# PRBonn/lidar_transfer

Hardware: AMD Instinct MI355X
Metric: Mrays/sec, one new ~1M-triangle mesh per scan -> 64x2048 range/label image (higher is better)
Workload: dtype f32; 1 GPU; C2: 64x2048 rays vs 999788-triangle synthetic scene (fov 3.0/-25.0); 1 step = 64 scans, each a new mesh; 48 scenes cycled; parallelism=scan-parallel x1, scans_in_flight=24, scans_per_call=8

## Files before the change

### lidar_transfer_amd/csrc/lt_api.hip

```cpp
#include "lt_internal.h"
#include <cpuid.h>
#include <stdarg.h>
#include <stdlib.h>
#include <string.h>

static thread_local char g_err[512] = "";

void lt_set_error(const char* fmt, ...) {
  va_list ap;
  va_start(ap, fmt);
  vsnprintf(g_err, sizeof(g_err), fmt, ap);
  va_end(ap);
}

int lt_cu_count(int device) {
  static int cache[64];
  const int slot = (device >= 0 && device < 64) ? device : 0;
  int v = __atomic_load_n(&cache[slot], __ATOMIC_RELAXED);
  if (v > 0) return v;
  hipDeviceProp_t prop;
  v = (hipGetDeviceProperties(&prop, device) == hipSuccess && prop.multiProcessorCount > 0) ? prop.multiProcessorCount : 256;
  __atomic_store_n(&cache[slot], v, __ATOMIC_RELAXED);
  return v;
}
// ... 77 lines not shown
  if (!out) {
    lt_set_error("lt_scene_create: NULL out pointer");
    return LT_ERR_INVALID_ARG;
  }
  *out = nullptr;
  if (device < 0) LT_HIP(hipGetDevice(&device));
  LT_HIP(hipSetDevice(device));
  lt_scene* s = (lt_scene*)calloc(1, sizeof(lt_scene));
  if (!s) {
    lt_set_error("lt_scene_create: out of host memory");
    return LT_ERR_NO_MEMORY;
  }
  s->device = device;
  int rc = dev_alloc(&s->partial, 6 * LT_BOUNDS_BLOCKS);
  if (rc == LT_OK) rc = dev_alloc(&s->params, 8);
  if (rc == LT_OK) rc = dev_alloc(&s->flags, 4);
  if (rc == LT_OK) rc = dev_alloc(&s->counters, 8 + 4 * LT_DBG_WAVES);
  if (rc == LT_OK && hipMemset(s->flags, 0, 4 * sizeof(unsigned)) != hipSuccess) rc = LT_ERR_HIP;
  for (int k = 0; rc == LT_OK && k < 10; ++k) {
    if (hipEventCreate(&s->ev[k]) != hipSuccess) {
      lt_set_error("hipEventCreate failed");
      rc = LT_ERR_HIP;
    } else {
      s->have_events = k + 1;
    }
  }
  if (rc != LT_OK) {
    lt_scene_destroy(s);
    return rc;
  }
  *out = s;
  return LT_OK;
}

extern "C" int lt_scene_destroy(lt_scene* s) {
  if (!s) return LT_OK;
  (void)hipSetDevice(s->device);
  (void)hipDeviceSynchronize();
  ws_free(s);
  if (s->owned_mesh) (void)hipFree(s->owned_mesh);
  if (s->partial) (void)hipFree(s->partial);
  if (s->params) (void)hipFree(s->params);
  if (s->flags) (void)hipFree(s->flags);
  if (s->counters) (void)hipFree(s->counters);
  if (s->overflow) (void)hipFree(s->overflow);
  if (s->tail_stack) (void)hipFree(s->tail_stack);
  if (s->tail_meta) (void)hipFree(s->tail_meta);
  if (s->tail_queue) (void)hipFree(s->tail_queue);
  if (s->tail_count) (void)hipFree(s->tail_count);
  if (s->sc_cell) (void)hipFree(s->sc_cell);
  if (s->sc_large) (void)hipFree(s->sc_large);
  if (s->sc_slices) (void)hipFree(s->sc_slices);
  if (s->sc_large_count) (void)hipFree(s->sc_large_count);
  for (int k = 0; k < s->have_events; ++k) (void)hipEventDestroy(s->ev[k]);
  free(s);
  return LT_OK;
}

int lt_check_mesh_args(const char* who, const void* verts, const void* faces, const void* colors,
                           const void* rem, int n_verts, int n_faces) {
  if (n_verts < 0 || n_faces < 0 || (n_faces > 0 && (!verts || !faces || !colors || !rem))) {
    lt_set_error("%s: invalid mesh (n_verts=%d n_faces=%d, NULL array?)", who, n_verts, n_faces);
    return LT_ERR_INVALID_ARG;
  }
  if (n_faces >= LT_MAX_FACES) {
    lt_set_error("%s: %d faces exceed LT_MAX_FACES", who, n_faces);
    return LT_ERR_TOO_LARGE;
  }
  return LT_OK;
}

extern "C" int lt_scene_set_mesh_dev(lt_scene* s, const float* verts, const int* faces, const int* colors,
                                     const float* rem, int n_verts, int n_faces) {
  if (!s) {
    lt_set_error("lt_scene_set_mesh_dev: NULL scene");
    return LT_ERR_INVALID_ARG;
  }
  LT_CHECK(lt_check_mesh_args("lt_scene_set_mesh_dev", verts, faces, colors, rem, n_verts, n_faces));
  s->verts = verts; s->faces = faces; s->colors = colors; s->rem = rem;
  s->n_verts = n_verts; s->n_faces = n_faces;
  s->built = 0;
  return LT_OK;
}

static size_t align256(size_t x) { return (x + 255) & ~(size_t)255; }

extern "C" int lt_scene_set_mesh_host(lt_scene* s, const float* verts, const int* faces, const int* colors,
                                      const float* rem, int n_verts, int n_faces, void* stream_) {
  if (!s) {
    lt_set_error("lt_scene_set_mesh_host: NULL scene");
    return LT_ERR_INVALID_ARG;
  }
  LT_CHECK(lt_check_mesh_args("lt_scene_set_mesh_host", verts, faces, colors, rem, n_verts, n_faces));
  hipStream_t stream = (hipStream_t)stream_;
  LT_HIP(hipSetDevice(s->device));
  const size_t bv = align256((size_t)n_verts * 12), bf = align256((size_t)n_faces * 12), bc = bv,
               br = align256((size_t)n_verts * 4);
  const size_t total = bv + bf + bc + br + 256;
  if (total > s->owned_mesh_bytes) {
    if (s->owned_mesh) {
      LT_HIP(hipDeviceSynchronize());
      (void)hipFree(s->owned_mesh);
      s->owned_mesh = nullptr;
      s->owned_mesh_bytes = 0;
    }
    LT_HIP(hipMalloc(&s->owned_mesh, total + total / 4));
// ... 156 lines not shown
```

### lidar_transfer_amd/csrc/lt_internal.h

```cpp
#pragma once
#include <hip/hip_runtime.h>
#include <stdint.h>
#include <stdio.h>
#include "lidarhip.h"

void lt_set_error(const char* fmt, ...);
int lt_cu_count(int device);

#define LT_HIP(call)                                                                          \
  do {                                                                                        \
    hipError_t e__ = (call);                                                                  \
    if (e__ != hipSuccess) {                                                                  \
      lt_set_error("%s failed: %s (%s:%d)", #call, hipGetErrorString(e__), __FILE__, __LINE__); \
      return e__ == hipErrorOutOfMemory ? LT_ERR_NO_MEMORY : LT_ERR_HIP;                      \
    }                                                                                         \
  } while (0)

#define LT_CHECK(expr)              \
  do {                              \
    int rc__ = (expr);              \
    if (rc__ != LT_OK) return rc__; \
  } while (0)

#define LT_FOR_MODEL(rows, sector, az, LAUNCH)                           \
// ... 7 lines not shown
                double fov_down_deg, int H, const double* sec, const double* az, int n_az, double* tab);
bool sector_ok(const char* who, double yaw_center, double span);
bool beam_azimuth_ok(const char* who, const double* az, int n);


#define LT_LEAF_MAX 4
#ifndef LT_SORT_TILE
#define LT_SORT_TILE 4096
#endif
#define LT_SORT_THREADS 256
#define LT_SEG_SUB 512
#define LT_STACK_LDS 32
#define LT_STACK_MAX 64
#define LT_STACK4_LDS 40
#define LT_STACK4_MAX 104
#define LT_TAIL_SAVE (LT_STACK4_MAX + 1)
#define LT_TAIL_STACK 512
#define LT_TAIL_DFS 256
#define LT_TRACE4_STEP_CAP 40

struct lt_scene {
  int device;
  const float* verts;
  const int* faces;
  const int* colors;
  const float* rem;
  int n_verts, n_faces;
  void* owned_mesh;
  size_t owned_mesh_bytes;
  int cap_faces;
  int np;
  uint32_t* keys[2];
  uint32_t* vals[2];
  uint32_t* hist;
  float4* tris;
  float4* seg;
  float4* nodes;
  float4* nodes4;
  float* partial;
  float* params;
  unsigned* flags;
  unsigned long long* counters;
  int* overflow;
  int cap_rays;
  int* tail_stack;
  float4* tail_meta;
  int* tail_queue;
  int* tail_count;
  int tail_parity;
  unsigned long long* sc_cell;
  int* sc_large;
  int2* sc_slices;
  int* sc_large_count;
  int sc_cap_cells, sc_cap_queue;
  int built;
  int sorted_buf;
  hipStream_t last_stream;
  hipEvent_t probe[2];
  hipEvent_t ev[10];
  int have_events;
  lt_stats stats;
};

struct lt_tsdf {
  int device;
  int dim[3];
  float origin[3];
  float voxel_size, trunc_margin;
  double voxel_size_d;
  double fov_up_deg, fov_down_deg;
  double bnds_given[6];
  size_t n;
  float *tsdf, *weight, *color, *rem;
  unsigned* col_epoch;
  unsigned* col_zw;
  unsigned epoch;
  int all_dirty;
  unsigned long long* bits;
  int* colinfo;
  float* colmax;
  int cap_w;
  int walk_w;
  float2* dct;
  size_t cap_dct;
  int n_obs;
  int wd_w;
  int wd_rho_bits, wd_n_quirk;
  float wd_qscale;
  int* wd_px;
  int* wd_start;
  int2* wd_ent;
  unsigned* wd_key;
  unsigned* wd_qcols;
  float4* rowtab;
  int rowtab_h;
  int rowtab_for_h;
  unsigned* zw_snap;
  unsigned* chunk_epoch;
  float4* obs4;
  size_t cap_obs4;
};

#define LT_BOUNDS_BLOCKS 256
#define LT_DBG_WAVES 16384
#define LT_FLAG_BAD_INDEX 1u
#define LT_FLAG_HIER_OVERFLOW 2u
#define LT_TRACE_DEBUG_STEPS 0x4000u
// ... 37 lines not shown
```

### lidar_transfer_amd/csrc/lt_scatter.hip

```cpp
#include "lt_internal.h"
#include <math.h>
#include <type_traits>
#include <stdlib.h>
#include <string.h>
#include "lt_normalize.h"

#define LT_PI_F 3.14159265358979f
#define LT_BIN_SLACK 4e-3f
#define LT_EMPTY_KEY 0xFFFFFFFFFFFFFFFFull

struct rs_params {
  int nb_az, nb_el;
  float az_scale;
  float az_off;
  float el_lo, el_scale;
  float dev_az, dev_el;
  float dev_fit[2];
  float el_c0, el_c1, az_c0, az_c1;
};

__device__ __forceinline__ float rs_az_off(float phi0, float az_scale) {
  if (!(phi0 == phi0)) return 0.f;
  const float x0 = (phi0 + LT_PI_F) * az_scale;
  return x0 - floorf(x0 + 0.5f);
}

__global__ __launch_bounds__(256) void k_rs_dirs(const float* __restrict__ rays, int n, unsigned flags,
                                                 float4* __restrict__ dirs, float2* __restrict__ ang,
                                                 float* __restrict__ partial) {
  __shared__ float red[4][2];
  float lo = INFINITY, hi = -INFINITY;
  for (int i = blockIdx.x * 256 + threadIdx.x; i < n; i += gridDim.x * 256) {
    const float rx = rays[3 * (size_t)i], ry = rays[3 * (size_t)i + 1], rz = rays[3 * (size_t)i + 2];
    const float D = (rx * rx + ry * ry) + rz * rz;
    const float r0 = lt_rsqrt_seed(D, flags);
    const float r = (1.5f * r0) + (((D * -0.5f) * r0) * (r0 * r0));
    const float dx = rx * r, dy = ry * r, dz = rz * r;
    dirs[i] = make_float4(dx, dy, dz, 0.f);
    const float phi = atan2f(dy, dx), th = atan2f(dz, sqrtf(dx * dx + dy * dy));
    ang[i] = make_float2(phi, th);
    if (th == th) { lo = fminf(lo, th); hi = fmaxf(hi, th); }
  }
#pragma unroll
  for (int o = 32; o > 0; o >>= 1) {
    lo = fminf(lo, __shfl_xor(lo, o, 64));
    hi = fmaxf(hi, __shfl_xor(hi, o, 64));
  }
  if ((threadIdx.x & 63) == 0) { red[threadIdx.x >> 6][0] = lo; red[threadIdx.x >> 6][1] = hi; }
  __syncthreads();
  if (threadIdx.x == 0) {
    partial[2 * blockIdx.x] = fminf(fminf(red[0][0], red[1][0]), fminf(red[2][0], red[3][0]));
    partial[2 * blockIdx.x + 1] = fmaxf(fmaxf(red[0][1], red[1][1]), fmaxf(red[2][1], red[3][1]));
  }
}
// ... 273 lines not shown
    n_tests += w >= 0 ? 1u : 0u;
    sc_hit<WIDE>(sc_mt(T, ox, oy, oz, g.x, g.y, g.z), w, face, cell);
  } else {
    for (int k = __float_as_int(g.x), e = __float_as_int(g.y); k < e; ++k) {
      const float4 d = *at<WIDE>(sdirs, (unsigned)k);
      ++n_tests;
      sc_hit<WIDE>(sc_mt(T, ox, oy, oz, d.x, d.y, d.z), __float_as_int(d.w), face, cell);
    }
  }
}

__global__ __launch_bounds__(256) void k_rs_sortdirs(const float4* __restrict__ dirs,
                                                     const uint32_t* __restrict__ bin_rays, int n,
                                                     float4* __restrict__ sdirs) {
  const int k = blockIdx.x * 256 + threadIdx.x;
  if (k >= n) return;
  const int ray = (int)bin_rays[k];
  float4 d = dirs[ray];
  d.w = __int_as_float(ray);
  sdirs[k] = d;
}

__global__ __launch_bounds__(256) void k_rs_grid(const int* __restrict__ bin_start,
                                                 const float4* __restrict__ sdirs, int nbins,
                                                 float4* __restrict__ grid) {
  const int b = blockIdx.x * 256 + threadIdx.x;
  if (b >= nbins) return;
  const int s = bin_start[b], e = bin_start[b + 1];
  float4 g = make_float4(0.f, 0.f, 0.f, __int_as_float(LT_GRID_EMPTY));
  if (e - s == 1) g = sdirs[s];
  else if (e - s > 1) g = make_float4(__int_as_float(s), __int_as_float(e), 0.f, __int_as_float(LT_GRID_MULTI));
  grid[b] = g;
}

#define LT_SC_BIG 512
#define LT_SC_CAP_SINGLE 1536
#define LT_SC_CAP_BATCH 8192
#ifndef LT_SC_SLICE
#define LT_SC_SLICE 512
#endif

#ifndef LT_SC_T
#define LT_SC_T 448
#endif
#define LT_SC_T2 (LT_SC_T - 256)
static_assert(LT_SC_T >= 256 && LT_SC_T <= 512 && LT_SC_T2 % 64 == 0, "LT_SC_T: 256, 320, 384, 448 or 512");

struct sc_shared {
  float4 q0[LT_SC_T], q1[LT_SC_T];
  float2 q2[LT_SC_T];
  unsigned pre[513];
  unsigned wsum[4];
  int kept;
};

struct sc_one { int cnt; unsigned a0; };

template <bool PUSH>
__device__ __forceinline__ sc_one sc_record_into(float4* s_q0, float4* s_q1, float2* s_q2, int slot, int f, const f3 A,
                                                 const f3 Bv, const f3 C, float ox, float oy, float oz, const rs_params& P,
                                                 int* __restrict__ large, int* __restrict__ large_count) {
  sc_one r;
  r.cnt = 0; r.a0 = 0;
  const float v0x = A.x, v0y = A.y, v0z = A.z, v1x = Bv.x, v1y = Bv.y, v1z = Bv.z;
  const float v2x = C.x, v2y = C.y, v2z = C.z;
  const float e1x = v1x - v0x, e1y = v1y - v0y, e2x = v2x - v0x, e2y = v2y - v0y;
  const bin_rect R = tri_bins(P, v0x - ox, v0y - oy, v0z - oz, v1x - ox, v1y - oy, v1z - oz, v2x - ox, v2y - oy,
                              v2z - oz, e1x, e1y, e2x, e2y);
  if (R.na > 0) {
    const int c32 = R.na * (R.e1 - R.e0 + 1);
    if (c32 > LT_SC_BIG) {
      if (PUSH) large[atomicAdd(large_count, 1)] = f;
    } else {
      r.cnt = c32;
      r.a0 = (unsigned)R.a0;
      s_q0[slot] = make_float4(v0x, v0y, v0z, e1x);
      s_q1[slot] = make_float4(e1y, v1z - v0z, e2x, e2y);
      s_q2[slot] = make_float2(v2z - v0z, __int_as_float((R.na - 1) | (R.e0 << 9)));
    }
  }
  return r;
}
template <bool PUSH>
__device__ __forceinline__ sc_one sc_record(sc_shared& S, int slot, int f, const f3 A, const f3 Bv, const f3 C, float ox,
                                            float oy, float oz, const rs_params& P, int* __restrict__ large,
                                            int* __restrict__ large_count) {
  return sc_record_into<PUSH>(S.q0, S.q1, S.q2, slot, f, A, Bv, C, ox, oy, oz, P, large, large_count);
}

template <bool PUSH, bool WIDE>
__device__ __forceinline__ void sc_setup(sc_shared& S, const float* __restrict__ verts, const int* __restrict__ faces,
                                         int n_verts, int n_faces, int first, float ox, float oy, float oz,
                                         const rs_params& P, int* __restrict__ large, int* __restrict__ large_count,
                                         unsigned* __restrict__ flags, sc_one& rA, sc_one& rB) {
  const int tid = threadIdx.x;
  rA.cnt = 0; rA.a0 = 0; rB.cnt = 0; rB.a0 = 0;
  const int fA = first + tid, fB = first + 256 + tid;
  const bool hasA = fA < n_faces, hasB = LT_SC_T2 > 0 && tid < LT_SC_T2 && fB < n_faces;
  if (n_verts <= 0) {
    if (PUSH && (hasA || hasB)) atomicOr(flags, LT_FLAG_BAD_INDEX);
    return;
  }
  const i3 iA = *at<WIDE>((const i3*)faces, (unsigned)(hasA ? fA : 0));
  i3 iB = iA;
  if (LT_SC_T2 > 0) iB = *at<WIDE>((const i3*)faces, (unsigned)(hasB ? fB : 0));
  const unsigned nv = (unsigned)n_verts;
  const bool okA = hasA && (unsigned)iA.x < nv && (unsigned)iA.y < nv && (unsigned)iA.z < nv;
// ... 99 lines not shown
    for (int u = 0; u < N; ++u) g[u] = *at<false>(grid, (unsigned)bin_of(cc[u], base[u], q2[u]));
    float th[N];
#pragma unroll
    for (int u = 0; u < N; ++u) {
      const bool act = cb + u * NT < c_end;
      const float4 q0 = ldq(s_q0, j4[u]), q1 = ldq(s_q1, j4[u]);
      tri_rec T;
      T.v0x = q0.x; T.v0y = q0.y; T.v0z = q0.z;
      T.e1x = q0.w; T.e1y = q1.x; T.e1z = q1.y;
      T.e2x = q1.z; T.e2y = q1.w; T.e2z = q2[u].x;
      const int w = __float_as_int(g[u].w);
      if (COUNT) n_cand += act ? 1u : 0u;
      n_tests += act && w >= 0 ? 1u : 0u;
      const float t = sc_mt(T, ox, oy, oz, g[u].x, g[u].y, g[u].z);
      th[u] = act && w != LT_GRID_MULTI ? t : NAN;
      if (act && w == LT_GRID_MULTI) sc_test_cell<WIDE>(T, first_face + (int)(j4[u] >> 2), g[u], sdirs, ox, oy, oz, cell, n_tests);
    }
#pragma unroll
    for (int u = 0; u < N; ++u) sc_hit<WIDE>(th[u], __float_as_int(g[u].w), first_face + (int)(j4[u] >> 2), cell);
  };
  for (int cb = c_begin + tix; cb < c_end; cb += PB * NT) {
    int live = 1;
#pragma unroll
    for (int u = 1; u < PB; ++u) live += __ballot(cb + u * NT < c_end) != 0ull ? 1 : 0;
    if constexpr (PB >= 4) {
      if (live == 4) { block(std::integral_constant<int, 4>{}, cb); continue; }
    }
    if constexpr (PB >= 3) {
      if (live == 3) { block(std::integral_constant<int, 3>{}, cb); continue; }
    }
    if constexpr (PB >= 2) {
      if (live == 2) { block(std::integral_constant<int, 2>{}, cb); continue; }
    }
    block(std::integral_constant<int, 1>{}, cb);
  }
}

template <bool COUNT>
__device__ __forceinline__ void sc_count(unsigned n_tests, unsigned n_cand, unsigned long long* __restrict__ counters) {
  if (COUNT) {
    unsigned long long vt = n_tests, vc = n_cand;
#pragma unroll
    for (int o = 32; o > 0; o >>= 1) { vt += __shfl_xor(vt, o, 64); vc += __shfl_xor(vc, o, 64); }
    if ((threadIdx.x & 63) == 0) { atomicAdd(&counters[1], vt); atomicAdd(&counters[0], vc); }
  }
}

#ifndef LT_SC_MAX_BATCH
#define LT_SC_MAX_BATCH 8
#endif
struct sc_job {
  const float* verts; const int* faces; const int* colors; const float* rem;
  rs_params P; const float4* grid; const float4* sdirs; const float4* dirs;
  unsigned long long* cell; int* large; int* large_count; int2* slices;
  unsigned* flags; unsigned long long* counters;
  float* endpoints; int* endcolors; float* range; float* endrem; int* tri;
  float ox, oy, oz;
  int n_verts, n_faces, n_rays, cap_slices;
  unsigned out_flags;
};
struct sc_batch {
  int n;
  int tris_blocks, resolve_blocks;
  int cap;
  int rest_blocks;
  int tris_block0[LT_SC_MAX_BATCH];
  int resolve_block0[LT_SC_MAX_BATCH];
  sc_job job[LT_SC_MAX_BATCH];
};
__device__ __forceinline__ int sc_find_job(const int (&block0)[LT_SC_MAX_BATCH], int block) {
  int j = 0;
#pragma unroll
  for (int k = 1; k < LT_SC_MAX_BATCH; ++k) j += block >= block0[k] ? 1 : 0;
  return j;
}


template <bool COUNT, bool WIDE>
__global__ __launch_bounds__(256) void k_sc_tris(const sc_batch B) {
  __shared__ sc_shared S;
  const int j = sc_find_job(B.tris_block0, (int)blockIdx.x);
  const sc_job& J = B.job[j];
  const int lb = (int)blockIdx.x - B.tris_block0[j];
  const int tid = threadIdx.x;
  const int first = lb * LT_SC_T;
  const rs_params P = J.P;
  const float ox = J.ox, oy = J.oy, oz = J.oz;
  sc_one rA, rB;
  sc_setup<true, WIDE>(S, J.verts, J.faces, J.n_verts, J.n_faces, first, ox, oy, oz, P, J.large, J.large_count, J.flags, rA,
                       rB);
  int total, preA, preB;
  sc_prefix(S, rA, rB, preA, preB, total);
  if (total < B.cap) {
    if (tid == 255) S.kept = total;
  } else {
    const bool crossA = preA < B.cap && preA + rA.cnt >= B.cap;
    const bool crossB = LT_SC_T2 > 0 && tid < LT_SC_T2 && preB < B.cap && preB + rB.cnt >= B.cap;
    if (crossA || crossB) {
      int kept = crossA ? preA + rA.cnt : preB + rB.cnt;
      const int n_sl = (total - kept + LT_SC_SLICE - 1) / LT_SC_SLICE;
      if (n_sl > 0) {
        const int base = atomicAdd(&J.large_count[1], n_sl);
        if (base + n_sl <= J.cap_slices) {
          for (int k = 0; k < n_sl; ++k) J.slices[base + k] = make_int2(lb, kept + k * LT_SC_SLICE);
        } else {
          atomicSub(&J.large_count[1], n_sl);
          kept = total;
        }
      }
      S.kept = kept;
    }
  }
  __syncthreads();
  const int kept = S.kept;
  unsigned n_tests = 0, n_cand = 0;
  sc_round_robin<COUNT, WIDE, 256, (LT_SC_T > 256 ? 512 : 256), LT_SC_PB>(S.pre, S.q0, S.q1, S.q2, P, J.grid, J.sdirs, J.cell,
                                                                          first, 0, kept, tid, ox, oy, oz, n_tests, n_cand);
  sc_count<COUNT>(n_tests, n_cand, J.counters);
}

#define LT_SC_REST_BLOCKS 512
#define LT_SC_REST_BLOCKS_BATCH 128
#define LT_SC_PARTS 8
template <bool COUNT, bool WIDE>
__global__ __launch_bounds__(256) void k_sc_rest(const sc_batch B) {
  __shared__ sc_shared S;
  const int rest_blocks = B.rest_blocks;
  const sc_job& J = B.job[blockIdx.x / rest_blocks];
  const int rb = blockIdx.x % rest_blocks;
  if (J.n_faces <= 0) return;
  const float* __restrict__ verts = J.verts;
  const int* __restrict__ faces = J.faces;
  const float4* __restrict__ grid = J.grid;
  const float4* __restrict__ sdirs = J.sdirs;
  unsigned long long* __restrict__ cell = J.cell;
  const float ox = J.ox, oy = J.oy, oz = J.oz;
  const rs_params P = J.P;
  const int n_large = J.large_count[0], n_slices = min(J.large_count[1], J.cap_slices);
  if (COUNT && rb == 0 && threadIdx.x == 0) J.counters[3] = (unsigned long long)n_large | ((unsigned long long)n_slices << 32);
  unsigned n_tests = 0, n_cand = 0;
  for (int q = rb; q < n_slices; q += rest_blocks) {
    const int2 sl = J.slices[q];
    const int first = sl.x * LT_SC_T;
    sc_one rA, rB;
    sc_setup<false, WIDE>(S, verts, faces, J.n_verts, J.n_faces, first, ox, oy, oz, P, nullptr, nullptr, nullptr, rA, rB);
    int total, preA, preB;
    sc_prefix(S, rA, rB, preA, preB, total);
    __syncthreads();
    sc_round_robin<COUNT, WIDE, 256, (LT_SC_T > 256 ? 512 : 256), LT_SC_PB_REST>(S.pre, S.q0, S.q1, S.q2, P, grid, sdirs, cell,
                                                                               first, sl.y, min(sl.y + LT_SC_SLICE, total),
                                                                               (int)threadIdx.x, ox, oy, oz, n_tests, n_cand);
    __syncthreads();
  }
  const int lane = threadIdx.x & 63;
  const int wave0 = rb * 4 + (threadIdx.x >> 6), nwaves = rest_blocks * 4;
  for (int v = wave0; v < n_large * LT_SC_PARTS; v += nwaves) {
    const int q = v / LT_SC_PARTS, part = v - q * LT_SC_PARTS;
    const int f = J.large[q];
    const float* pa = verts + 3 * (size_t)faces[3 * (size_t)f];
    const float* pb = verts + 3 * (size_t)faces[3 * (size_t)f + 1];
    const float* pc = verts + 3 * (size_t)faces[3 * (size_t)f + 2];
    tri_rec T;
    T.v0x = pa[0]; T.v0y = pa[1]; T.v0z = pa[2];
    const float v1x = pb[0], v1y = pb[1], v1z = pb[2], v2x = pc[0], v2y = pc[1], v2z = pc[2];
    T.e1x = v1x - T.v0x; T.e1y = v1y - T.v0y; T.e1z = v1z - T.v0z;
    T.e2x = v2x - T.v0x; T.e2y = v2y - T.v0y; T.e2z = v2z - T.v0z;
    const bin_rect R = tri_bins(P, T.v0x - ox, T.v0y - oy, T.v0z - oz, v1x - ox, v1y - oy, v1z - oz, v2x - ox,
                                v2y - oy, v2z - oz, T.e1x, T.e1y, T.e2x, T.e2y);
    const int total = R.na > 0 ? R.na * (R.e1 - R.e0 + 1) : 0;
    const int parts = min(max((total + 1023) / 1024, 1), LT_SC_PARTS);
    if (part >= parts) continue;
    for (int w = part * 64 + lane; w < total; w += 64 * parts) {
      const int row = w / R.na;
      const int e = R.e0 + row;
      int az = R.a0 + (w - row * R.na);
      if (az >= P.nb_az) az -= P.nb_az;
      if (COUNT) ++n_cand;
      sc_test_cell<WIDE>(T, f, grid[e * P.nb_az + az], sdirs, ox, oy, oz, cell, n_tests);
    }
  }
  sc_count<COUNT>(n_tests, n_cand, J.counters);
}

template <bool COUNT>
__global__ __launch_bounds__(256) void k_sc_resolve(const sc_batch B) {
  const int j = sc_find_job(B.resolve_block0, (int)blockIdx.x);
  const sc_job& J = B.job[j];
  const int ray = ((int)blockIdx.x - B.resolve_block0[j]) * 256 + threadIdx.x;
  unsigned long long* __restrict__ cell = J.cell;
  const int* __restrict__ faces = J.faces;
  float* __restrict__ endpoints = J.endpoints;
  int* __restrict__ endcolors = J.endcolors;
  float* __restrict__ range = J.range;
  float* __restrict__ endrem = J.endrem;
  int* __restrict__ tri_out = J.tri;
  const unsigned flags = J.out_flags;
  if (ray == 0) { J.large_count[0] = 0; J.large_count[1] = 0; }
  bool hit = false;
  if (ray < J.n_rays) {
    const unsigned long long key = cell[ray];
    const float4 d = J.dirs[ray];
    cell[ray] = LT_EMPTY_KEY;
    hit = key != LT_EMPTY_KEY;
    if (hit) {
      const float t = __uint_as_float((unsigned)(key >> 32));
      const int face = (int)(unsigned)(key & 0xFFFFFFFFull);
      const int i0 = faces[3 * (size_t)face], i1 = faces[3 * (size_t)face + 1], i2 = faces[3 * (size_t)face + 2];
      const int* __restrict__ colors = J.colors;
      const float* __restrict__ rem = J.rem;
      const bool label = (flags & LT_TRACE_LABEL_IMAGE) != 0;
      int c0 = 0, c1 = 0, c2 = 0;
      float r0 = 0.f, r1 = 0.f, r2 = 0.f;
      if (endcolors) {
        c2 = colors[3 * (size_t)i0 + 2];
        if (!label) { c0 = colors[3 * (size_t)i0]; c1 = colors[3 * (size_t)i0 + 1]; }
      }
      if (endrem) { r0 = rem[i0]; r1 = rem[i1]; r2 = rem[i2]; }
      if (endpoints) {
        endpoints[3 * (size_t)ray] = J.ox + d.x * t;
        endpoints[3 * (size_t)ray + 1] = J.oy + d.y * t;
        endpoints[3 * (size_t)ray + 2] = J.oz + d.z * t;
      }
      if (endcolors) {
        if (label) {
          endcolors[ray] = (int)(float)c2;
        } else {
          endcolors[3 * (size_t)ray] = (int)(float)c0;
          endcolors[3 * (size_t)ray + 1] = (int)(float)c1;
          endcolors[3 * (size_t)ray + 2] = (int)(float)c2;
        }
      }
      if (endrem) endrem[ray] = ((r0 + r1) + r2) / 3.0f;
      if (range) range[ray] = t;
      if (tri_out) tri_out[ray] = face;
    } else if (flags & LT_TRACE_WRITE_MISSES) {
      if (endpoints) { endpoints[3 * (size_t)ray] = 0.f; endpoints[3 * (size_t)ray + 1] = 0.f; endpoints[3 * (size_t)ray + 2] = 0.f; }
      if (endcolors) {
        if (flags & LT_TRACE_LABEL_IMAGE) endcolors[ray] = 0;
        else { endcolors[3 * (size_t)ray] = 0; endcolors[3 * (size_t)ray + 1] = 0; endcolors[3 * (size_t)ray + 2] = 0; }
      }
      if (endrem) endrem[ray] = 0.f;
      if (range) range[ray] = 0.f;
      if (tri_out) tri_out[ray] = -1;
    }
  }
  if (COUNT) {
    unsigned long long vh = hit ? 1u : 0u;
#pragma unroll
    for (int o = 32; o > 0; o >>= 1) vh += __shfl_xor(vh, o, 64);
    if ((threadIdx.x & 63) == 0) atomicAdd(&J.counters[2], vh);
// ... 93 lines not shown
    free(r);
    return rc;
  }
  if (hipMemsetAsync(r->prm, 0, sizeof(rs_params), stream) != hipSuccess) {
    lt_set_error("%s: hipMemsetAsync failed", who);
    rs_free(r);
    free(r);
    return LT_ERR_HIP;
  }
  hipLaunchKernelGGL(k_rs_dirs, dim3(256), dim3(256), 0, stream, rays, n, r->norm_flags, r->dirs, r->ang, r->partial);
  const int refit = grid_az > 0 ? 0 : 1;
  if (refit) hipLaunchKernelGGL(k_rs_fit, dim3(64), dim3(256), 0, stream, r->ang, n, r->nb_az, r->prm);
  hipLaunchKernelGGL(k_rs_keys, dim3((n + 255) / 256 > 0 ? (n + 255) / 256 : 1), dim3(256), 0, stream, r->ang, n,
                     r->nb_az, r->nb_el, refit, r->partial, r->prm, r->keys[0], r->vals[0]);
  int buf = 0;
  if (n > 0) lt_sort_pairs(r->keys, r->vals, r->hist, n, 30, stream, &buf);
  r->bin_rays = r->vals[buf];
  hipLaunchKernelGGL(k_rs_starts, dim3((n + 1 + 255) / 256), dim3(256), 0, stream, r->keys[buf], n, (int)nbins,
                     r->bin_start);
  if (n > 0)
    hipLaunchKernelGGL(k_rs_sortdirs, dim3((n + 255) / 256), dim3(256), 0, stream, r->dirs, r->bin_rays, n, r->sdirs);
  hipLaunchKernelGGL(k_rs_grid, dim3((unsigned)((nbins + 255) / 256)), dim3(256), 0, stream, r->bin_start, r->sdirs,
                     (int)nbins, r->grid);
  const hipError_t le = hipGetLastError();
  if (le != hipSuccess) {
    lt_set_error("%s: kernel launch failed: %s", who, hipGetErrorString(le));
    (void)hipStreamSynchronize(stream);
    rs_free(r);
    free(r);
    return LT_ERR_HIP;
  }
  if (hipStreamSynchronize(stream) != hipSuccess ||
      hipMemcpy(&r->prm_host, r->prm, sizeof(rs_params), hipMemcpyDeviceToHost) != hipSuccess) {
    lt_set_error("%s: ray set preparation failed: %s", who, hipGetErrorString(hipGetLastError()));
    rs_free(r);
    free(r);
    return LT_ERR_HIP;
  }
  rs_derive(r->prm_host);
  *out = r;
  return LT_OK;
}

extern "C" int lt_rayset_create_dev(lt_rayset** out, const float* rays, int n_rays, int height, unsigned flags,
                                    void* stream) {
  return rs_create("lt_rayset_create_dev", out, rays, n_rays, height, 0, 0, flags, stream);
}

extern "C" int lt_rayset_create_grid_dev(lt_rayset** out, const float* rays, int n_rays, int height, int nb_az, int nb_el,
                                         unsigned flags, void* stream) {
  return rs_create("lt_rayset_create_grid_dev", out, rays, n_rays, height, nb_az, nb_el, flags, stream);
}

static int sc_reserve(lt_scene* s, int n_faces, int n_rays, hipStream_t stream) {
  if (!s->sc_large_count) {
    LT_HIP(hipMalloc((void**)&s->sc_large_count, 4 * sizeof(int)));
    LT_HIP(hipMemsetAsync(s->sc_large_count, 0, 4 * sizeof(int), stream));
  }
  if (n_rays > s->sc_cap_cells) {
    if (s->sc_cell) {
      LT_HIP(hipDeviceSynchronize());
      (void)hipFree(s->sc_cell);
      s->sc_cell = nullptr;
      s->sc_cap_cells = 0;
    }
    LT_HIP(hipMalloc((void**)&s->sc_cell, (size_t)n_rays * sizeof(unsigned long long)));
    s->sc_cap_cells = n_rays;
    LT_HIP(hipMemsetAsync(s->sc_cell, 0xFF, (size_t)n_rays * sizeof(unsigned long long), stream));
  }
  if (n_faces > s->sc_cap_queue) {
    if (s->sc_large || s->sc_slices) {
      LT_HIP(hipDeviceSynchronize());
      (void)hipFree(s->sc_large);
      (void)hipFree(s->sc_slices);
      s->sc_large = nullptr;
      s->sc_slices = nullptr;
      s->sc_cap_queue = 0;
    }
    const size_t cap = (size_t)n_faces + n_faces / 4 + 1024;
    LT_HIP(hipMalloc((void**)&s->sc_large, cap * sizeof(int)));
    LT_HIP(hipMalloc((void**)&s->sc_slices, cap * sizeof(int2)));
    s->sc_cap_queue = (int)cap;
  }
  return LT_OK;
}

struct sc_item {
  lt_scene* s;
  lt_rayset* r;
  const float* origin;
  float* endpoints; int* endcolors; float* range; float* endrem; int* tri;
};

static int sc_launch_batch(const sc_item* it, int n_items, unsigned flags, hipStream_t stream, bool count,
                           lt_scene* probe) {
  sc_batch B;
  memset(&B, 0, sizeof(B));
  for (int k = 0; k < LT_SC_MAX_BATCH; ++k) B.tris_block0[k] = B.resolve_block0[k] = 0x7fffffff;
  static const bool force_wide = getenv("LIDARHIP_FORCE_WIDE") != nullptr;
  bool wide = force_wide;
  int tb = 0, rb = 0;
  for (int i = 0; i < n_items; ++i) {
    lt_scene* s = it[i].s;
    lt_rayset* r = it[i].r;
    const int n = s->n_faces, R = r->n_rays;
    if (R <= 0) continue;
    LT_CHECK(sc_reserve(s, n, R, stream));
    sc_job& J = B.job[B.n++];
    J.verts = s->verts; J.faces = s->faces; J.colors = s->colors; J.rem = s->rem;
    J.P = r->prm_host; J.grid = r->grid; J.sdirs = r->sdirs; J.dirs = r->dirs;
    J.cell = s->sc_cell; J.large = s->sc_large; J.large_count = s->sc_large_count; J.slices = s->sc_slices;
    J.flags = s->flags; J.counters = s->counters;
    J.endpoints = it[i].endpoints; J.endcolors = it[i].endcolors; J.range = it[i].range; J.endrem = it[i].endrem;
    J.tri = it[i].tri;
    J.ox = it[i].origin[0]; J.oy = it[i].origin[1]; J.oz = it[i].origin[2];
    J.n_verts = s->n_verts; J.n_faces = n; J.n_rays = R; J.cap_slices = s->sc_cap_queue;
    J.out_flags = flags;
    B.tris_block0[B.n - 1] = tb;
    B.resolve_block0[B.n - 1] = rb;
    tb += (n + LT_SC_T - 1) / LT_SC_T;
    rb += (R + 255) / 256;
    wide = wide || (size_t)n * 12 >= (1ull << 32) || (size_t)s->n_verts * 12 >= (1ull << 32) ||
           (size_t)R * 16 >= (1ull << 32);
  }
  if (B.n == 0) return LT_OK;
  B.tris_blocks = tb;
  B.resolve_blocks = rb;
  static const int env_cap = []() {
    const char* e = getenv("LIDARHIP_SC_CAP");
    return e ? atoi(e) : 0;
  }();
  B.cap = env_cap > 0 ? env_cap : (n_items > 1 ? LT_SC_CAP_BATCH : LT_SC_CAP_SINGLE);
  static const int env_rest = []() {
    const char* e = getenv("LIDARHIP_SC_REST_BLOCKS");
    return e ? atoi(e) : 0;
  }();
  B.rest_blocks = env_rest > 0 ? env_rest : (n_items > 1 ? LT_SC_REST_BLOCKS_BATCH : LT_SC_REST_BLOCKS);
  const dim3 b(256);
#define SC_LAUNCH(KERNEL, GRID) \
  do { \
    if (count && wide) hipLaunchKernelGGL((KERNEL<true, true>), GRID, b, 0, stream, B); \
    else if (count) hipLaunchKernelGGL((KERNEL<true, false>), GRID, b, 0, stream, B); \
    else if (wide) hipLaunchKernelGGL((KERNEL<false, true>), GRID, b, 0, stream, B); \
    else hipLaunchKernelGGL((KERNEL<false, false>), GRID, b, 0, stream, B); \
  } while (0)
  if (tb > 0) {
    if (probe && probe->probe[0]) LT_HIP(hipEventRecord(probe->probe[0], stream));
    SC_LAUNCH(k_sc_tris, dim3(tb));
    if (probe) {
      if (probe->probe[1]) LT_HIP(hipEventRecord(probe->probe[1], stream));
      probe->probe[0] = probe->probe[1] = nullptr;
    }
    SC_LAUNCH(k_sc_rest, dim3(B.n * B.rest_blocks));
  }
#undef SC_LAUNCH
  if (count) hipLaunchKernelGGL(k_sc_resolve<true>, dim3(rb), b, 0, stream, B);
  else hipLaunchKernelGGL(k_sc_resolve<false>, dim3(rb), b, 0, stream, B);
  LT_HIP(hipGetLastError());
  return LT_OK;
}

extern "C" int lt_scene_render_dev(lt_scene* s, lt_rayset* r, const float* origin, float* endpoints, int* endcolors,
                                   float* range, float* endrem, int* tri, unsigned flags, void* stream_,
                                   lt_stats* stats) {
  if (!s || !r || !origin) {
    lt_set_error("lt_scene_render_dev: NULL scene / rayset / origin");
    return LT_ERR_INVALID_ARG;
  }
  if (s->device != r->device) {
    lt_set_error("lt_scene_render_dev: scene on device %d, rayset on device %d", s->device, r->device);
    return LT_ERR_INVALID_ARG;
  }
  hipStream_t stream = (hipStream_t)stream_;
  LT_HIP(hipSetDevice(s->device));
  s->last_stream = stream;
  const int n = s->n_faces, R = r->n_rays;
  const bool timed = stats != nullptr, count = (flags & LT_TRACE_COUNT) != 0;
  s->stats.n_rays = R;
  s->stats.n_faces = n;
  if (R > 0) {
    if (count) LT_HIP(hipMemsetAsync(s->counters, 0, 4 * sizeof(unsigned long long), stream));
    if (timed) LT_HIP(hipEventRecord(s->ev[7], stream));
    const sc_item it = {s, r, origin, endpoints, endcolors, range, endrem, tri};
    LT_CHECK(sc_launch_batch(&it, 1, flags, stream, count, count ? nullptr : s));
    if (timed) LT_HIP(hipEventRecord(s->ev[8], stream));
  }
  if (timed || count) {
    LT_HIP(hipStreamSynchronize(stream));
    if (timed && R > 0) LT_HIP(hipEventElapsedTime(&s->stats.ms_trace, s->ev[7], s->ev[8]));
    if (count && R > 0) {
      unsigned long long c[4];
      LT_HIP(hipMemcpy(c, s->counters, sizeof(c), hipMemcpyDeviceToHost));
      s->stats.nodes_visited = c[0];
      s->stats.tris_tested = c[1];
      s->stats.n_hits = (int)c[2];
      s->stats.stack_overflows = 0;
      s->stats.entries_culled = 0;
    }
    if (stats) *stats = s->stats;
  }
  return LT_OK;
}

extern "C" int lt_scene_render_batch_dev(int n_scans, lt_scene* const* scenes, lt_rayset* const* raysets,
                                         const float* origins, float* const* endpoints, int* const* endcolors,
                                         float* const* range, float* const* endrem, int* const* tri, unsigned flags,
                                         void* stream_) {
  if (n_scans < 0 || n_scans > LT_SC_MAX_BATCH || (n_scans > 0 && (!scenes || !raysets || !origins))) {
    lt_set_error("lt_scene_render_batch_dev: invalid argument (n_scans=%d, at most %d per call)", n_scans,
                 LT_SC_MAX_BATCH);
    return LT_ERR_INVALID_ARG;
  }
  if (flags & LT_TRACE_COUNT) {
    lt_set_error("lt_scene_render_batch_dev: LT_TRACE_COUNT is a single-scan diagnostic (lt_scene_render_dev)");
    return LT_ERR_INVALID_ARG;
  }
  if (n_scans == 0) return LT_OK;
  hipStream_t stream = (hipStream_t)stream_;
  sc_item it[LT_SC_MAX_BATCH];
  lt_scene* probe = nullptr;
  for (int i = 0; i < n_scans; ++i) {
    if (!scenes[i] || !raysets[i] || scenes[i]->device != raysets[i]->device ||
        scenes[i]->device != scenes[0]->device) {
      lt_set_error("lt_scene_render_batch_dev: scan %d: NULL scene / rayset, or not all on one device", i);
      return LT_ERR_INVALID_ARG;
    }
    for (int k = 0; k < i; ++k)
      if (scenes[k] == scenes[i]) {
        lt_set_error("lt_scene_render_batch_dev: scans %d and %d are the same scene (a scene renders one scan at a time)", k, i);
        return LT_ERR_INVALID_ARG;
      }
    it[i] = {scenes[i], raysets[i], origins + 3 * i, endpoints ? endpoints[i] : nullptr,
             endcolors ? endcolors[i] : nullptr, range ? range[i] : nullptr, endrem ? endrem[i] : nullptr,
             tri ? tri[i] : nullptr};
    scenes[i]->last_stream = stream;
    scenes[i]->stats.n_rays = raysets[i]->n_rays;
    scenes[i]->stats.n_faces = scenes[i]->n_faces;
    if (!probe && scenes[i]->probe[0]) probe = scenes[i];
  }
  LT_HIP(hipSetDevice(scenes[0]->device));
  return sc_launch_batch(it, n_scans, flags, stream, false, probe ? probe : scenes[0]);
}

extern "C" int lt_debug_scatter_queues(lt_scene* s, int* out2) {
  if (!s || !out2) return LT_ERR_INVALID_ARG;
  LT_HIP(hipSetDevice(s->device));
  LT_HIP(hipDeviceSynchronize());
  unsigned long long c = 0;
  LT_HIP(hipMemcpy(&c, s->counters + 3, sizeof(c), hipMemcpyDeviceToHost));
  out2[0] = (int)(c & 0xFFFFFFFFull);
  out2[1] = (int)(c >> 32);
  return LT_OK;
}
extern "C" int lt_debug_scatter_large(lt_scene* s, int* out, int n) {
  if (!s || !out || n < 0 || n > s->sc_cap_queue) return LT_ERR_INVALID_ARG;
  LT_HIP(hipSetDevice(s->device));
  LT_HIP(hipDeviceSynchronize());
  LT_HIP(hipMemcpy(out, s->sc_large, (size_t)n * sizeof(int), hipMemcpyDeviceToHost));
  return LT_OK;
}
extern "C" int lt_debug_rayset_params(lt_rayset* r, int* nb, float* p) {
  if (!r || !nb || !p) return LT_ERR_INVALID_ARG;
  const rs_params& P = r->prm_host;
  nb[0] = P.nb_az; nb[1] = P.nb_el;
  p[0] = P.az_scale; p[1] = P.az_off; p[2] = P.el_lo; p[3] = P.el_scale; p[4] = P.dev_az; p[5] = P.dev_el;
  return LT_OK;
}
```

Baseline: 11680 Mrays/s.

## Spill scatter tile setup to global memory so rest slices skip recomputation

When a triangle tile overflows the per-block capacity and is split into slices, the first kernel now copies its computed LDS setup state (queues and prefix sums) into a global spill slot. The slot index is packed into the slice descriptor. Rest-stage blocks then reload that state straight into LDS with global_load_lds instead of rerunning sc_setup and the prefix scan for every slice. This costs extra global writes and reads per large tile and a bounded pool of spill slots, with a fallback to recomputation when the pool runs out.

```diff
diff --git a/lidar_transfer_amd/csrc/lt_api.hip b/lidar_transfer_amd/csrc/lt_api.hip
--- a/lidar_transfer_amd/csrc/lt_api.hip
+++ b/lidar_transfer_amd/csrc/lt_api.hip
@@ -153,6 +153,7 @@
   if (s->sc_large) (void)hipFree(s->sc_large);
   if (s->sc_slices) (void)hipFree(s->sc_slices);
   if (s->sc_large_count) (void)hipFree(s->sc_large_count);
+  if (s->sc_spill) (void)hipFree(s->sc_spill);
   for (int k = 0; k < s->have_events; ++k) (void)hipEventDestroy(s->ev[k]);
   free(s);
   return LT_OK;
diff --git a/lidar_transfer_amd/csrc/lt_internal.h b/lidar_transfer_amd/csrc/lt_internal.h
--- a/lidar_transfer_amd/csrc/lt_internal.h
+++ b/lidar_transfer_amd/csrc/lt_internal.h
@@ -83,7 +83,8 @@
   int* sc_large;
   int2* sc_slices;
   int* sc_large_count;
-  int sc_cap_cells, sc_cap_queue;
+  float4* sc_spill;
+  int sc_cap_cells, sc_cap_queue, sc_spill_slots;
   int built;
   int sorted_buf;
   hipStream_t last_stream;
diff --git a/lidar_transfer_amd/csrc/lt_scatter.hip b/lidar_transfer_amd/csrc/lt_scatter.hip
--- a/lidar_transfer_amd/csrc/lt_scatter.hip
+++ b/lidar_transfer_amd/csrc/lt_scatter.hip
@@ -1,5 +1,6 @@
 #include "lt_internal.h"
 #include <math.h>
+#include <stddef.h>
 #include <type_traits>
 #include <stdlib.h>
 #include <string.h>
@@ -379,7 +380,20 @@
   unsigned pre[513];
   unsigned wsum[4];
   int kept;
+  int slot;
 };
+static_assert(sizeof(sc_shared) <= 20480, "sc_shared: 20 KB of LDS = 8 workgroups per CU");
+
+#define LT_SC_SPILL_VEC ((int)((offsetof(sc_shared, pre) + 513 * sizeof(unsigned) + 15) / 16))
+#define LT_SC_SPILL_PER_LANE ((LT_SC_SPILL_VEC + 255) / 256)
+#define LT_SC_SPILL_SLOTS 64
+#define LT_SC_SPILL_SLOTS_MAX 4096
+static_assert(offsetof(sc_shared, q0) == 0 && offsetof(sc_shared, q1) == sizeof(float4) * LT_SC_T &&
+              offsetof(sc_shared, q2) == 2 * sizeof(float4) * LT_SC_T &&
+              offsetof(sc_shared, pre) == 2 * sizeof(float4) * LT_SC_T + sizeof(float2) * LT_SC_T,
+              "the spilled arrays are the contiguous head of sc_shared");
+static_assert((size_t)LT_SC_SPILL_VEC * 16 <= sizeof(sc_shared), "a spill unit stays inside sc_shared");
+static_assert((size_t)LT_SC_T * LT_SC_BIG <= (1u << 18), "first candidate of a slice: 18 bits");
 
 struct sc_one { int cnt; unsigned a0; };
 
@@ -585,7 +599,7 @@
 struct sc_job {
   const float* verts; const int* faces; const int* colors; const float* rem;
   rs_params P; const float4* grid; const float4* sdirs; const float4* dirs;
-  unsigned long long* cell; int* large; int* large_count; int2* slices;
+  unsigned long long* cell; int* large; int* large_count; int2* slices; float4* spill;
   unsigned* flags; unsigned long long* counters;
   float* endpoints; int* endcolors; float* range; float* endrem; int* tri;
   float ox, oy, oz;
@@ -597,6 +611,7 @@
   int tris_blocks, resolve_blocks;
   int cap;
   int rest_blocks;
+  int spill_slots;
   int tris_block0[LT_SC_MAX_BATCH];
   int resolve_block0[LT_SC_MAX_BATCH];
   sc_job job[LT_SC_MAX_BATCH];
@@ -625,27 +640,43 @@
   int total, preA, preB;
   sc_prefix(S, rA, rB, preA, preB, total);
   if (total < B.cap) {
-    if (tid == 255) S.kept = total;
+    if (tid == 255) { S.kept = total; S.slot = -1; }
   } else {
     const bool crossA = preA < B.cap && preA + rA.cnt >= B.cap;
     const bool crossB = LT_SC_T2 > 0 && tid < LT_SC_T2 && preB < B.cap && preB + rB.cnt >= B.cap;
     if (crossA || crossB) {
       int kept = crossA ? preA + rA.cnt : preB + rB.cnt;
+      int slot = -1;
       const int n_sl = (total - kept + LT_SC_SLICE - 1) / LT_SC_SLICE;
       if (n_sl > 0) {
         const int base = atomicAdd(&J.large_count[1], n_sl);
         if (base + n_sl <= J.cap_slices) {
-          for (int k = 0; k < n_sl; ++k) J.slices[base + k] = make_int2(lb, kept + k * LT_SC_SLICE);
+          if (B.spill_slots > 0) {
+            slot = atomicAdd(&J.large_count[2], 1);
+            if (slot >= B.spill_slots) slot = -1;
+          }
+          for (int k = 0; k < n_sl; ++k) J.slices[base + k] = make_int2(lb, (kept + k * LT_SC_SLICE) | ((slot + 1) << 18));
         } else {
           atomicSub(&J.large_count[1], n_sl);
           kept = total;
         }
       }
       S.kept = kept;
+      S.slot = slot;
     }
   }
   __syncthreads();
   const int kept = S.kept;
+  const int slot = S.slot;
+  if (slot >= 0) {
+    const float4* src = (const float4*)&S;
+    float4* dst = J.spill + (size_t)slot * LT_SC_SPILL_VEC;
+#pragma unroll
+    for (int k = 0; k < LT_SC_SPILL_PER_LANE; ++k) {
+      const int i = tid + 256 * k;
+      if (i < LT_SC_SPILL_VEC) dst[i] = src[i];
+    }
+  }
   unsigned n_tests = 0, n_cand = 0;
   sc_round_robin<COUNT, WIDE, 256, (LT_SC_T > 256 ? 512 : 256), LT_SC_PB>(S.pre, S.q0, S.q1, S.q2, P, J.grid, J.sdirs, J.cell,
                                                                           first, 0, kept, tid, ox, oy, oz, n_tests, n_cand);
@@ -670,18 +701,41 @@
   const float ox = J.ox, oy = J.oy, oz = J.oz;
   const rs_params P = J.P;
   const int n_large = J.large_count[0], n_slices = min(J.large_count[1], J.cap_slices);
-  if (COUNT && rb == 0 && threadIdx.x == 0) J.counters[3] = (unsigned long long)n_large | ((unsigned long long)n_slices << 32);
+  if (COUNT && rb == 0 && threadIdx.x == 0) {
+    J.counters[3] = (unsigned long long)n_large | ((unsigned long long)n_slices << 32);
+    J.counters[4] = (unsigned long long)min(J.large_count[2], B.spill_slots);
+  }
   unsigned n_tests = 0, n_cand = 0;
   for (int q = rb; q < n_slices; q += rest_blocks) {
-    const int2 sl = J.slices[q];
+    const int2 sl_v = J.slices[q];
+    const int2 sl = make_int2(__builtin_amdgcn_readfirstlane(sl_v.x), __builtin_amdgcn_readfirstlane(sl_v.y));
     const int first = sl.x * LT_SC_T;
-    sc_one rA, rB;
-    sc_setup<false, WIDE>(S, verts, faces, J.n_verts, J.n_faces, first, ox, oy, oz, P, nullptr, nullptr, nullptr, rA, rB);
-    int total, preA, preB;
-    sc_prefix(S, rA, rB, preA, preB, total);
-    __syncthreads();
+    const int c0 = sl.y & ((1 << 18) - 1), slot = (sl.y >> 18) - 1;
+    int total;
+    if (slot >= 0) {
+      const float4* src = J.spill + (size_t)slot * LT_SC_SPILL_VEC;
+      int t = (int)threadIdx.x;
+      asm volatile("" : "+v"(t));
+      t &= 255;
+      float4* dst = (float4*)&S + (t & ~63);
+#pragma unroll
+      for (int k = 0; k < LT_SC_SPILL_PER_LANE; ++k) {
+        const int i = t + 256 * k;
+        if (i < LT_SC_SPILL_VEC)
+          __builtin_amdgcn_global_load_lds((const __attribute__((address_space(1))) void*)(src + i),
+                                           (__attribute__((address_space(3))) void*)(dst + 256 * k), 16, 0, 0);
+      }
+      __syncthreads();
+      total = (int)(S.pre[LT_SC_T] >> 13);
+    } else {
+      sc_one rA, rB;
+      sc_setup<false, WIDE>(S, verts, faces, J.n_verts, J.n_faces, first, ox, oy, oz, P, nullptr, nullptr, nullptr, rA, rB);
+      int preA, preB;
+      sc_prefix(S, rA, rB, preA, preB, total);
+      __syncthreads();
+    }
     sc_round_robin<COUNT, WIDE, 256, (LT_SC_T > 256 ? 512 : 256), LT_SC_PB_REST>(S.pre, S.q0, S.q1, S.q2, P, grid, sdirs, cell,
-                                                                               first, sl.y, min(sl.y + LT_SC_SLICE, total),
+                                                                               first, c0, min(c0 + LT_SC_SLICE, total),
                                                                                (int)threadIdx.x, ox, oy, oz, n_tests, n_cand);
     __syncthreads();
   }
@@ -728,7 +782,7 @@
   float* __restrict__ endrem = J.endrem;
   int* __restrict__ tri_out = J.tri;
   const unsigned flags = J.out_flags;
-  if (ray == 0) { J.large_count[0] = 0; J.large_count[1] = 0; }
+  if (ray == 0) { J.large_count[0] = 0; J.large_count[1] = 0; J.large_count[2] = 0; }
   bool hit = false;
   if (ray < J.n_rays) {
     const unsigned long long key = cell[ray];
@@ -928,10 +982,14 @@
   return rs_create("lt_rayset_create_grid_dev", out, rays, n_rays, height, nb_az, nb_el, flags, stream);
 }
 
-static int sc_reserve(lt_scene* s, int n_faces, int n_rays, hipStream_t stream) {
+static int sc_reserve(lt_scene* s, int n_faces, int n_rays, int spill_slots, hipStream_t stream) {
   if (!s->sc_large_count) {
     LT_HIP(hipMalloc((void**)&s->sc_large_count, 4 * sizeof(int)));
     LT_HIP(hipMemsetAsync(s->sc_large_count, 0, 4 * sizeof(int), stream));
+  }
+  if (spill_slots > s->sc_spill_slots) {
+    LT_HIP(hipMalloc((void**)&s->sc_spill, (size_t)spill_slots * LT_SC_SPILL_VEC * sizeof(float4)));
+    s->sc_spill_slots = spill_slots;
   }
   if (n_rays > s->sc_cap_cells) {
     if (s->sc_cell) {
@@ -975,17 +1033,25 @@
   for (int k = 0; k < LT_SC_MAX_BATCH; ++k) B.tris_block0[k] = B.resolve_block0[k] = 0x7fffffff;
   static const bool force_wide = getenv("LIDARHIP_FORCE_WIDE") != nullptr;
   bool wide = force_wide;
+  static const int spill_slots = []() {
+    const char* on = getenv("LIDARHIP_SC_SPILL");
+    if (on && atoi(on) == 0) return 0;
+    const char* e = getenv("LIDARHIP_SC_SPILL_SLOTS");
+    const int n = e ? atoi(e) : LT_SC_SPILL_SLOTS;
+    return n < 0 ? 0 : (n > LT_SC_SPILL_SLOTS_MAX ? LT_SC_SPILL_SLOTS_MAX : n);
+  }();
   int tb = 0, rb = 0;
   for (int i = 0; i < n_items; ++i) {
     lt_scene* s = it[i].s;
     lt_rayset* r = it[i].r;
     const int n = s->n_faces, R = r->n_rays;
     if (R <= 0) continue;
-    LT_CHECK(sc_reserve(s, n, R, stream));
+    LT_CHECK(sc_reserve(s, n, R, spill_slots, stream));
     sc_job& J = B.job[B.n++];
     J.verts = s->verts; J.faces = s->faces; J.colors = s->colors; J.rem = s->rem;
     J.P = r->prm_host; J.grid = r->grid; J.sdirs = r->sdirs; J.dirs = r->dirs;
     J.cell = s->sc_cell; J.large = s->sc_large; J.large_count = s->sc_large_count; J.slices = s->sc_slices;
+    J.spill = s->sc_spill;
     J.flags = s->flags; J.counters = s->counters;
     J.endpoints = it[i].endpoints; J.endcolors = it[i].endcolors; J.range = it[i].range; J.endrem = it[i].endrem;
     J.tri = it[i].tri;
@@ -1012,6 +1078,7 @@
     return e ? atoi(e) : 0;
   }();
   B.rest_blocks = env_rest > 0 ? env_rest : (n_items > 1 ? LT_SC_REST_BLOCKS_BATCH : LT_SC_REST_BLOCKS);
+  B.spill_slots = spill_slots;
   const dim3 b(256);
 #define SC_LAUNCH(KERNEL, GRID) \
   do { \
@@ -1055,7 +1122,7 @@
   s->stats.n_rays = R;
   s->stats.n_faces = n;
   if (R > 0) {
-    if (count) LT_HIP(hipMemsetAsync(s->counters, 0, 4 * sizeof(unsigned long long), stream));
+    if (count) LT_HIP(hipMemsetAsync(s->counters, 0, 5 * sizeof(unsigned long long), stream));
     if (timed) LT_HIP(hipEventRecord(s->ev[7], stream));
     const sc_item it = {s, r, origin, endpoints, endcolors, range, endrem, tri};
     LT_CHECK(sc_launch_batch(&it, 1, flags, stream, count, count ? nullptr : s));
@@ -1128,6 +1195,15 @@
   out2[1] = (int)(c >> 32);
   return LT_OK;
 }
+extern "C" int lt_debug_scatter_spills(lt_scene* s, int* out) {
+  if (!s || !out) return LT_ERR_INVALID_ARG;
+  LT_HIP(hipSetDevice(s->device));
+  LT_HIP(hipDeviceSynchronize());
+  unsigned long long c = 0;
+  LT_HIP(hipMemcpy(&c, s->counters + 4, sizeof(c), hipMemcpyDeviceToHost));
+  *out = (int)c;
+  return LT_OK;
+}
 extern "C" int lt_debug_scatter_large(lt_scene* s, int* out, int n) {
   if (!s || !out || n < 0 || n > s->sc_cap_queue) return LT_ERR_INVALID_ARG;
   LT_HIP(hipSetDevice(s->device));
```

Result: no change. 11700 Mrays/s (median of 6 runs) (+0.2%).
